# westlake-moonlight/vision_transformer_detector

Hardware: AMD Instinct MI355X
Metric: images/sec ViT-B/16 detector fwd, batch 256, 1/2/4/8 MI355X; MFMA util % (higher is better)
Workload: dtype bf16; 1 GPU; vit_b16_224 detector forward + decode; per_gpu_batch=256, global_batch=256, parallelism=dp1, streams_per_gpu=2, hip_graph=False

## Files before the change

### vision_transformer_detector_amd/csrc/vtd_gemm.hip

```cpp
#include <stdlib.h>

#include <algorithm>
#include <mutex>
#include <type_traits>

#include "vtd_common.h"
#include "vtd_gemm_epi.h"
#include "vtd_launch.h"

namespace vtd {

namespace {

constexpr int BM = 128, BN = 128, KB = 128;
constexpr int NT = 256;
constexpr int TILE_BYTES = BM * KB;


__device__ __forceinline__ int swz(int row, int chunk) {
  return row * KB + ((chunk ^ (row & 7)) << 4);
}


__device__ __forceinline__ void gload4(i32x4 (&ra)[4], i32x4 (&rb)[4], const char* ga,
// ... 166 lines not shown
#pragma unroll
        for (int cb = 0; cb < 2; ++cb) {
          const int r = 16 * cb + fr, c = 4 * (sb & 1) + g;
          const bf16x8 b = *reinterpret_cast<const bf16x8*>(smem + (sb >> 1) * 4096 + r * 128 +
                                                            ((c ^ (r & 7)) << 4));
          acc[cb] = __builtin_amdgcn_mfma_f32_16x16x32_bf16(__builtin_bit_cast(bf16x8, a[j]), b,
                                                            acc[cb], 0, 0, 0);
        }
      }
    }
  };
  for (int s0 = 0; s0 < nks; s0 += 2 * SK_CH) {
    if (s0 + SK_CH < nks) load(a1, s0 + SK_CH);
    compute(a0, s0);
    if (s0 + 2 * SK_CH < nks) load(a0, s0 + 2 * SK_CH);
    if (s0 + SK_CH < nks) compute(a1, s0 + SK_CH);
  }
#pragma unroll
  for (int cb = 0; cb < 2; ++cb)
#pragma unroll
    for (int r = 0; r < 4; ++r) epi_store(e, M, N, m0 + 4 * g + r, n0 + 16 * cb + fr, acc[cb][r]);
}

constexpr int BBM = 256, BBN = 256, BNT = 512;
#ifndef VTD_TRS
#define VTD_TRS 0
#endif
#ifndef VTD_PP2_PH
#define VTD_PP2_PH 2
#endif
constexpr int BSTAGE = (BBM + BBN) * KB;
static_assert(8 * 32 * 68 * 4 + 8 * 128 * 8 <= 2 * BSTAGE,
              "epilogue staging + LayerNorm-fold row tables must fit the stages");

typedef __attribute__((address_space(3))) void lds_void_t;
typedef __attribute__((address_space(1))) const void gbl_void_t;


struct NoPF {
  __device__ void operator()() const {}
};

template <int O0, int O1, int O2, int O3>
__device__ __forceinline__ void lds_read4_b64(const void* p, float2 (&o)[4]) {
  const uint32_t a = static_cast<uint32_t>(reinterpret_cast<uintptr_t>(p));
  asm volatile(
      "ds_read_b64 %0, %4 offset:%5\n\tds_read_b64 %1, %4 offset:%6\n\t"
      "ds_read_b64 %2, %4 offset:%7\n\tds_read_b64 %3, %4 offset:%8\n\ts_waitcnt lgkmcnt(0)"
      : "=v"(o[0]), "=v"(o[1]), "=v"(o[2]), "=v"(o[3])
      : "v"(a), "i"(O0), "i"(O1), "i"(O2), "i"(O3)
      : "memory");
}
__device__ __forceinline__ void store_s3(const EpiArgs& e, int64_t idx, const i32x4& o, f32x4 v0,
                                         f32x4 v1) {
  const i32x4 lo = {(int)pack_lo_bf16x2(v0[0], v0[1], (uint32_t)o[0]),
                    (int)pack_lo_bf16x2(v0[2], v0[3], (uint32_t)o[1]),
                    (int)pack_lo_bf16x2(v1[0], v1[1], (uint32_t)o[2]),
                    (int)pack_lo_bf16x2(v1[2], v1[3], (uint32_t)o[3])};
  bf16_t* p = static_cast<bf16_t*>(e.out) + idx;
  store_out16(p + e.s3, lo);
}
template <int EPI, int PR = 32, int DG = 0, typename PF = NoPF, bool TRL = false>
__device__ __forceinline__ void epilogue_fast(const f32x4 (&acc)[8][4], float* ep, int lane,
                                              int m_base, int n_base, const EpiArgs& e,
                                              const float2* lst = nullptr, PF pf = PF{}) {
  constexpr int ACT = EPI & 3;
  constexpr bool OUT_BF16 = (EPI & 4) != 0;
  constexpr bool RESID = (EPI & 8) != 0 && !(DG & 2);
  constexpr bool NOBIAS = (EPI & EPI_PARTIAL) != 0;
  constexpr bool LNF = (EPI & EPI_LNF) != 0, STAT = (EPI & EPI_STAT) != 0 && !(DG & 1);
  constexpr bool F8O = (EPI & EPI_F8O) != 0;
  auto sidx = [](int row, int col) { return row * 64 + (((col >> 2) ^ (row & 7)) << 2) + (col & 3); };
  constexpr int NB = PR / 16;
  constexpr int NIT = PR / 8;
  const int fr = lane & 15, fg = lane >> 4;
  const int c8 = (lane & 7) * 8, rsub = lane >> 3;
  f32x4 b0 = {}, b1 = {};
  if constexpr (!NOBIAS) {
    b0 = *reinterpret_cast<const f32x4*>(e.bias + n_base + c8);
    b1 = *reinterpret_cast<const f32x4*>(e.bias + n_base + c8 + 4);
  }
  f32x4 cs0 = {}, cs1 = {};
  if constexpr (LNF) {
    cs0 = *reinterpret_cast<const f32x4*>(e.colsum + n_base + c8);
    cs1 = *reinterpret_cast<const f32x4*>(e.colsum + n_base + c8 + 4);
  }
  constexpr bool RPRE = RESID && OUT_BF16;
  i32x4 rraw[2][NIT];
  auto load_raw = [&](int pp, i32x4 (&dst)[NIT]) {
#pragma unroll
    for (int it = 0; it < NIT; ++it) {
      const int64_t m = m_base + pp * PR + it * 8 + rsub;
      dst[it] = *reinterpret_cast<const i32x4*>(static_cast<const bf16_t*>(e.resid) + m * e.ldr +
                                                n_base + c8);
    }
  };
  if constexpr (RPRE) load_raw(0, rraw[0]);
  else pf();
#pragma unroll
  for (int p = 0; p < 128 / PR; ++p) {
    if constexpr (TRL) {
#pragma unroll
      for (int i = 0; i < NB; ++i)
#pragma unroll
        for (int jj = 0; jj < 4; ++jj)
          *reinterpret_cast<f32x4*>(ep + sidx(i * 16 + fr, 32 * (jj >> 1) + 8 * fg + 4 * (jj & 1))) =
              acc[p * NB + i][jj];
    } else {
#pragma unroll
      for (int i = 0; i < NB; ++i)
#pragma unroll
        for (int j = 0; j < 4; ++j)
#pragma unroll
          for (int r2 = 0; r2 < 4; ++r2)
            ep[sidx(i * 16 + fg * 4 + r2, j * 16 + fr)] = acc[p * NB + i][j][r2];
    }
    if constexpr (RPRE) {
      if (p + 1 < 128 / PR) load_raw(p + 1, rraw[(p + 1) & 1]);
      if (p == 0) pf();
    }
    constexpr bool ASM_ST = LNF && !std::is_same<PF, NoPF>::value;
    float2 stv[4];
    if constexpr (ASM_ST) {
      static_assert(PR == 32, "the fold's table reads assume 32-row passes");
      if (p == 0) lds_read4_b64<0, 64, 128, 192>(lst + rsub, stv);
      else if (p == 1) lds_read4_b64<256, 320, 384, 448>(lst + rsub, stv);
      else if (p == 2) lds_read4_b64<512, 576, 640, 704>(lst + rsub, stv);
      else lds_read4_b64<768, 832, 896, 960>(lst + rsub, stv);
    }
    f32x4 rv[NIT][2];
    [[maybe_unused]] float2 stkeep = float2{0.f, 0.f};
    if constexpr (RESID && !RPRE) {
#pragma unroll
      for (int it = 0; it < NIT; ++it) {
        const int64_t m = m_base + p * PR + it * 8 + rsub;
        load_resid8<OUT_BF16>(e, m * e.ldr + n_base + c8, rv[it][0], rv[it][1]);
      }
    }
#pragma unroll
    for (int it = 0; it < NIT; ++it) {
      const int row = it * 8 + rsub;
      f32x4 v0 = *reinterpret_cast<const f32x4*>(ep + sidx(row, c8));
      f32x4 v1 = *reinterpret_cast<const f32x4*>(ep + sidx(row, c8 + 4));
      if constexpr (ASM_ST) epi_lnfold8_st(stv[it], cs0, cs1, v0, v1);
      else if constexpr (LNF) epi_lnfold8_st(lst[p * PR + row], cs0, cs1, v0, v1);
      v0 += b0;
      v1 += b1;
      if constexpr ((EPI & EPI_RA) != 0) epi_rowadd8(e, m_base + p * PR + row, n_base + c8, v0, v1);
      act_ct8<ACT>(v0, v1);
      if constexpr (RPRE) {
        const i32x4 w = rraw[p & 1][it];
        v0 += bf16x4_to_f32((uint32_t)w[0], (uint32_t)w[1]);
        v1 += bf16x4_to_f32((uint32_t)w[2], (uint32_t)w[3]);
      } else if constexpr (RESID) {
        v0 += rv[it][0];
        v1 += rv[it][1];
      }
      if constexpr ((EPI & EPI_O2) != 0) epi_out2_8(e, m_base + p * PR + row, n_base + c8, v0, v1);
      const int64_t idx = (int64_t)(m_base + p * PR + row) * e.ldo + n_base + c8;
      if constexpr (OUT_BF16) {
        if constexpr (F8O) {
          bf16_round4(v0);
          bf16_round4(v1);
          float am = 0.f;
#pragma unroll
          for (int j = 0; j < 4; ++j) am = fmaxf(am, fmaxf(fabsf(v0[j]), fabsf(v1[j])));
          am = fmaxf(am, dpp_f32<0xB1>(am));
          am = fmaxf(am, dpp_f32<0x4E>(am));
          const int E = mx8_exponent(am);
          const float inv = __uint_as_float((uint32_t)(127 - E) << 23);
          const uint2 qv = {mx8_pack4(v0[0], v0[1], v0[2], v0[3], inv),
                            mx8_pack4(v1[0], v1[1], v1[2], v1[3], inv)};
          *reinterpret_cast<uint2*>(static_cast<uint8_t*>(e.out) + idx) = qv;
          if ((lane & 3) == 0) {
            const int n = n_base + c8, b = n >> 5;
            e.sout[((int64_t)(b >> 2) * e.s_rows + m_base + p * PR + row) * 4 + (b & 3)] =
                (uint8_t)(E + 127);
          }
          continue;
        }
        const i32x4 o = {(int)pack_bf16x2(v0[0], v0[1]), (int)pack_bf16x2(v0[2], v0[3]),
                         (int)pack_bf16x2(v1[0], v1[1]), (int)pack_bf16x2(v1[2], v1[3])};
        if constexpr (DG & 4) asm volatile("" ::"v"(o));
        else store_out16(static_cast<bf16_t*>(e.out) + idx, o);
        if constexpr ((EPI & EPI_S3) != 0) store_s3(e, idx, o, v0, v1);
        if constexpr (STAT) {
          f32x2 pv[4];
          bf16x8_unpack(o, pv);
          const float mean = sum8_dpp(pairs_sum(pv)) * (1.f / 64.f);
          const float m2 = sum8_dpp(pairs_m2(pv, mean));
          if ((lane & 7) == it) stkeep = float2{mean, m2};
        }
      } else {
        float* op = static_cast<float*>(e.out) + idx;
        *reinterpret_cast<f32x4*>(op) = v0;
        *reinterpret_cast<f32x4*>(op + 4) = v1;
      }
    }
    if constexpr (OUT_BF16 && STAT && !F8O) {
      static_assert(NIT <= 8, "one statistics row per lane of an 8-lane group");
      if ((lane & 7) < NIT)
        e.statout[(int64_t)(n_base >> 6) * e.stat_ld + m_base + p * PR + (lane & 7) * 8 + rsub] =
            stkeep;
    }
  }
}
template <int PR = 32>
__device__ __forceinline__ void epilogue_generic_pass(const float* ep, int lane, int M, int N,
                                                      int m_base, int n_base, const EpiArgs& e) {
  constexpr int ES = 68;
#pragma unroll 1
  for (int it = 0; it < PR / 4; ++it) {
    const int row = it * 4 + (lane >> 4), col = (lane & 15) * 4;
    const f32x4 v = *reinterpret_cast<const f32x4*>(ep + row * ES + col);
    epi_store4(e, M, N, m_base + row, n_base + col, v);
  }
}
// ... 247 lines not shown
    else pp_mfma<4, 2, F32>(acc, a, b1);
    if constexpr (!NB) pp_barrier();
    if constexpr (n2) {
      pp2_issue<2, AW>(smem, src, wave, kt + 2, kt & 1);
      pp2_issue<3, AW>(smem, src, wave, kt + 2, kt & 1);
      asm volatile("s_waitcnt vmcnt(10)" ::: "memory");
    } else {
      asm volatile("s_waitcnt vmcnt(0)" ::: "memory");
    }
    if constexpr (!NB) pp_barrier();
    if constexpr (TR) pp_mfma_t<4, 0, F32>(acc, a, b0);
    else pp_mfma<4, 0, F32>(acc, a, b0);
    if constexpr (!NB) pp_barrier();
  };
  int kt = 0;
  for (; kt + 2 < nk; ++kt) step(kt, std::true_type{}, std::true_type{});
  if (kt + 1 < nk) step(kt++, std::true_type{}, std::false_type{});
  step(kt, std::false_type{}, std::false_type{});
  if (wm == 0) pp_barrier();
}

template <int I0, bool TR, bool F32>
__device__ __forceinline__ void pp_mfma32(f32x4 (&acc)[8][4], const bf16x8 (&a)[4][2],
                                          const bf16x8 (&b0)[2][2], const bf16x8 (&b1)[2][2]) {
  if constexpr (TR) {
    pp_mfma_t<I0, 0, F32>(acc, a, b0);
    pp_mfma_t<I0, 2, F32>(acc, a, b1);
  } else {
    pp_mfma<I0, 0, F32>(acc, a, b0);
    pp_mfma<I0, 2, F32>(acc, a, b1);
  }
}

template <bool AW>
__device__ __forceinline__ void pp2_issue_first(char* smem, const PP2Src<AW>& src, int nk,
                                                int wave) {
  pp2_issue<0, AW>(smem, src, wave, 0, 0);
  pp2_issue<2, AW>(smem, src, wave, 0, 0);
  pp2_issue<3, AW>(smem, src, wave, 0, 0);
  pp2_issue<1, AW>(smem, src, wave, 0, 0);
  if (nk > 1) {
    pp2_issue<0, AW>(smem, src, wave, 1, 1);
    pp2_issue<2, AW>(smem, src, wave, 1, 1);
    pp2_issue<3, AW>(smem, src, wave, 1, 1);
  }
}

template <bool TR, bool F32 = false, bool AW = true, int EX = 0>
__device__ __forceinline__ void pp2_mainloop_2ph(f32x4 (&acc)[8][4], char* smem,
                                                 const PP2Src<AW>& src, int nk, int wave, int wm,
                                                 int wn, int fr, int fg,
                                                 uint64_t* t_prologue = nullptr) {
  if (nk > 1) asm volatile("s_waitcnt vmcnt(%0)" ::"i"(6 + EX) : "memory");
  else asm volatile("s_waitcnt vmcnt(%0)" ::"i"(EX) : "memory");
  pp_barrier();
  if (t_prologue) *t_prologue = __builtin_amdgcn_s_memtime();
  if (wm == 1) pp_barrier();
  const int ra = wm * 64, rb = wn * 32;
  bf16x8 a[4][2], b0[2][2], b1[2][2];
  auto step = [&](int kt, auto t1, auto t2, auto ex) {
    const char* st = smem + (kt & 1) * BSTAGE;
    constexpr bool n1 = decltype(t1)::value, n2 = decltype(t2)::value;
    constexpr int W8 = 8 + decltype(ex)::value;
    pp_load_a(a, st + 0 * 16384, ra, fr, fg);
    if constexpr (TR) {
      pp_load_b_t(b0, st + 2 * 16384, rb, fr, fg);
// ... 4 lines not shown
    }
    if constexpr (n1) {
      pp2_issue<1, AW>(smem, src, wave, kt + 1, (kt + 1) & 1);
      asm volatile("s_waitcnt vmcnt(%0)" ::"i"(W8) : "memory");
    } else {
      asm volatile("s_waitcnt vmcnt(0)" ::: "memory");
    }
    pp_barrier();
    pp_mfma32<0, TR, F32>(acc, a, b0, b1);
    pp_barrier();
    pp_load_a(a, st + 1 * 16384, ra, fr, fg);
    if constexpr (n2) {
      pp2_issue<0, AW>(smem, src, wave, kt + 2, kt & 1);
      pp2_issue<2, AW>(smem, src, wave, kt + 2, kt & 1);
      pp2_issue<3, AW>(smem, src, wave, kt + 2, kt & 1);
      asm volatile("s_waitcnt vmcnt(%0)" ::"i"(W8) : "memory");
    } else {
      asm volatile("s_waitcnt vmcnt(0) lgkmcnt(0)" ::: "memory");
    }
    pp_barrier();
    pp_mfma32<4, TR, F32>(acc, a, b0, b1);
    if (n1 || n2 || wm == 0) pp_barrier();
  };
  constexpr std::integral_constant<int, 0> ex0{};
  int kt = 0;
  if constexpr (EX > 0) {
    if (nk > 2) step(kt++, std::true_type{}, std::true_type{}, std::integral_constant<int, EX>{});
  }
  for (; kt + 2 < nk; ++kt) step(kt, std::true_type{}, std::true_type{}, ex0);
  if (kt + 1 < nk) step(kt++, std::true_type{}, std::false_type{}, ex0);
  step(kt, std::false_type{}, std::false_type{}, ex0);
}

template <int EPI, int DG = 0, typename PF = NoPF>
__device__ __forceinline__ void epilogue_direct(const f32x4 (&acc)[8][4], int lane, int m_base,
                                                int n_base, const EpiArgs& e,
                                                const float2* lst = nullptr, PF pf = PF{}) {
  constexpr int ACT = EPI & 3;
  constexpr bool OUT_BF16 = (EPI & 4) != 0;
  constexpr bool RESID = (EPI & 8) != 0 && !(DG & 2);
  constexpr bool LNF = (EPI & EPI_LNF) != 0, STAT = (EPI & EPI_STAT) != 0 && !(DG & 1);
  constexpr bool F8O = (EPI & EPI_F8O) != 0;
  static_assert(!(F8O && (STAT || (EPI & EPI_S3) != 0)), "MX-fp8 output: no statistics / split");
  const int fr = lane & 15, fg = lane >> 4;
  f32x4 bias[2][2], cs[2][2] = {};
#pragma unroll
  for (int jp = 0; jp < 2; ++jp)
#pragma unroll
    for (int h = 0; h < 2; ++h) {
      bias[jp][h] = *reinterpret_cast<const f32x4*>(e.bias + n_base + 32 * jp + 8 * fg + 4 * h);
      if constexpr (LNF)
        cs[jp][h] = *reinterpret_cast<const f32x4*>(e.colsum + n_base + 32 * jp + 8 * fg + 4 * h);
    }
  constexpr bool RPRE = RESID && OUT_BF16;
  i32x4 rraw[2][4][2];
  auto load_raw = [&](int h0, i32x4 (&dst)[4][2]) {
#pragma unroll
    for (int i = 0; i < 4; ++i)
#pragma unroll
      for (int jp = 0; jp < 2; ++jp)
        dst[i][jp] = *reinterpret_cast<const i32x4*>(
            static_cast<const bf16_t*>(e.resid) + (int64_t)(m_base + 16 * (h0 + i) + fr) * e.ldr +
            n_base + 32 * jp + 8 * fg);
  };
  if constexpr (RPRE) load_raw(0, rraw[0]);
  else pf();
#pragma unroll
  for (int i0 = 0; i0 < 8; i0 += 4) {
    f32x4 rv[4][2][2];
    float2 st[4];
    if constexpr (LNF && !std::is_same<PF, NoPF>::value) {
      if (i0 == 0) lds_read4_b64<0, 128, 256, 384>(lst + fr, st);
      else lds_read4_b64<512, 640, 768, 896>(lst + fr, st);
    } else if constexpr (LNF) {
#pragma unroll
      for (int i = 0; i < 4; ++i) st[i] = lst[16 * (i0 + i) + fr];
    }
    [[maybe_unused]] float2 stkeep = float2{0.f, 0.f};
    if constexpr (RPRE) {
      if (i0 == 0) {
        load_raw(4, rraw[1]);
        pf();
      }
    } else if constexpr (RESID) {
#pragma unroll
      for (int i = 0; i < 4; ++i)
#pragma unroll
        for (int jp = 0; jp < 2; ++jp) {
          load_resid8<OUT_BF16>(e, (int64_t)(m_base + 16 * (i0 + i) + fr) * e.ldr + n_base +
                                       32 * jp + 8 * fg, rv[i][jp][0], rv[i][jp][1]);
        }
    }
#pragma unroll
    for (int i = 0; i < 4; ++i) {
      float tsum = 0.f;
      i32x4 ob[2];
#pragma unroll
      for (int jp = 0; jp < 2; ++jp) {
        f32x4 v0 = acc[i0 + i][2 * jp];
// ... 8 lines not shown
        if constexpr (RPRE) {
          const i32x4 w = rraw[i0 >> 2][i][jp];
          v0 += bf16x4_to_f32((uint32_t)w[0], (uint32_t)w[1]);
          v1 += bf16x4_to_f32((uint32_t)w[2], (uint32_t)w[3]);
        } else if constexpr (RESID) {
          v0 += rv[i][jp][0];
          v1 += rv[i][jp][1];
        }
        if constexpr ((EPI & EPI_O2) != 0) epi_out2_8(e, mrow, ncol, v0, v1);
        const int64_t idx = (int64_t)mrow * e.ldo + ncol;
        if constexpr (F8O) {
          bf16_round4(v0);
          bf16_round4(v1);
          float am = 0.f;
#pragma unroll
          for (int j = 0; j < 4; ++j) am = fmaxf(am, fmaxf(fabsf(v0[j]), fabsf(v1[j])));
          am = xmax32(xmax16(am));
          const int E = mx8_exponent(am);
          const float inv = __uint_as_float((uint32_t)(127 - E) << 23);
          const uint2 qv = {mx8_pack4(v0[0], v0[1], v0[2], v0[3], inv),
                            mx8_pack4(v1[0], v1[1], v1[2], v1[3], inv)};
          *reinterpret_cast<uint2*>(static_cast<uint8_t*>(e.out) + idx) = qv;
          if (fg == 0) {
            const int b = (n_base + 32 * jp) >> 5;
            e.sout[((int64_t)(b >> 2) * e.s_rows + mrow) * 4 + (b & 3)] = (uint8_t)(E + 127);
          }
          continue;
        }
        if constexpr (OUT_BF16) {
          const i32x4 o = {(int)pack_bf16x2(v0[0], v0[1]), (int)pack_bf16x2(v0[2], v0[3]),
                           (int)pack_bf16x2(v1[0], v1[1]), (int)pack_bf16x2(v1[2], v1[3])};
          if constexpr (DG & 4) asm volatile("" ::"v"(o));
          else store_out16(static_cast<bf16_t*>(e.out) + idx, o);
          if constexpr ((EPI & EPI_S3) != 0) store_s3(e, idx, o, v0, v1);
          if constexpr (STAT) {
            ob[jp] = o;
            tsum += bf16x8_sum(o);
          }
        } else {
          float* op = static_cast<float*>(e.out) + idx;
          *reinterpret_cast<f32x4*>(op) = v0;
          *reinterpret_cast<f32x4*>(op + 4) = v1;
        }
      }
      if constexpr (OUT_BF16 && STAT) {
        const float mean = xsum32(xsum16(tsum)) * (1.f / 64.f);
        const float m2 = xsum32(xsum16(bf16x8_m2(ob[0], mean) + bf16x8_m2(ob[1], mean)));
        if (fg == i) stkeep = float2{mean, m2};
      }
    }
    if constexpr (OUT_BF16 && STAT)
      e.statout[(int64_t)(n_base >> 6) * e.stat_ld + m_base + 16 * (i0 + fg) + fr] = stkeep;
  }
}

__device__ __forceinline__ void epilogue_direct_generic(const f32x4 (&acc)[8][4], float* ep,
                                                        int lane, int M, int N, int m_base,
                                                        int n_base, const EpiArgs& e) {
  constexpr int ES = 68;
  const int fr = lane & 15, fg = lane >> 4;
#pragma unroll
  for (int p = 0; p < 4; ++p) {
#pragma unroll
    for (int i = 0; i < 2; ++i)
#pragma unroll
      for (int jj = 0; jj < 4; ++jj)
        *reinterpret_cast<f32x4*>(ep + (i * 16 + fr) * ES + 32 * (jj >> 1) + 8 * fg +
                                  4 * (jj & 1)) = acc[p * 2 + i][jj];
    epilogue_generic_pass<32>(ep, lane, M, N, m_base + p * 32, n_base, e);
  }
}

#if VTD_DIAG
constexpr int kStampSlots = 16384;
__device__ uint64_t g_pp2_stamps[kStampSlots * 6];
#endif

template <int EPI, bool TR = false, int DG = 0>
__global__ __launch_bounds__(BNT) void gemm_tn_bf16_pp2_kernel(
    int M, int N, int K, const bf16_t* __restrict__ A, int lda,
    const bf16_t* __restrict__ Bt, int ldb, int tiles_m, int tiles_n, EpiArgs e, int ksplit) {
  extern __shared__ __attribute__((aligned(16))) char smem[];
  const int tid = threadIdx.x;
  const int lane = tid & 63;
  const int wave = __builtin_amdgcn_readfirstlane(tid >> 6);
  const int wm = wave >> 2, wn = wave & 3;
  uint64_t ts[4] = {0, 0, 0, 0};
  [[maybe_unused]] uint64_t rt0 = 0;
  if constexpr ((DG & 16) != 0) {
    ts[0] = __builtin_amdgcn_s_memtime();
    rt0 = __builtin_amdgcn_s_memrealtime();
  }
  asm volatile("" ::"s"(M), "s"(N), "s"(K), "s"(A), "s"(lda), "s"(Bt), "s"(ldb), "s"(tiles_m),
               "s"(tiles_n), "s"(ksplit), "s"(e.to.tiles_n), "s"(e.to.grouped), "s"(e.aw));
  const int nt = tiles_m * tiles_n, nwg = nt * ksplit;
  const int bid = blockIdx.x;
#if VTD_DIAG
  if (e.dsl > 0 && bid < 256 && ((bid >> 3) & 1))
    for (int i = 0; i < e.dsl; ++i) __builtin_amdgcn_s_sleep(8);
#endif
  const int xcd = bid & 7, q = nwg >> 3, r = nwg & 7;
  const int v = xcd * q + min(xcd, r) + (bid >> 3);
  const int split = ksplit > 1 ? v / nt : 0, tile = v - split * nt;
  int tm, tn;
  tile_coords(tile, e.to, tm, tn);
  const int m0 = tm * BBM, n0 = tn * BBN;
  const int nk_all = K / 64, nks = ksplit > 1 ? (nk_all + ksplit - 1) / ksplit : nk_all;
  const int k0 = split * nks, nk = min(nks, nk_all - k0);
  PP2Src<pp2_wraps(EPI)> src;
  pp2b_sources<TR>(src, A, lda, M, Bt, ldb, N, m0, n0, wave, lane, k0 * 64, true, e.aw);
  constexpr bool kEarly = VTD_PP2_PH == 2 && (DG & 32) == 0;
  constexpr bool kLnf = EPI != EPI_GENERIC && (EPI & EPI_LNF) != 0;
  if constexpr (kEarly) {
    pp2_issue_first(smem, src, nk, wave);
    __builtin_amdgcn_sched_barrier(0);
    asm volatile("" ::: "memory");
  }
  if (ksplit > 1) e.out = static_cast<float*>(e.out) + split * e.split_stride;
  float2 lst[2] = {float2{0.f, 0.f}, float2{0.f, 0.f}};
  if constexpr (kLnf) {
    lst[0] = e.lnstat[min(m0 + wm * 128 + lane, M - 1)];
    lst[1] = e.lnstat[min(m0 + wm * 128 + 64 + lane, M - 1)];
  }
  f32x4 acc[8][4];
#pragma unroll
  for (int i = 0; i < 8; ++i)
#pragma unroll
    for (int j = 0; j < 4; ++j) {
      acc[i][j] = f32x4{0.f, 0.f, 0.f, 0.f};
      if constexpr (kEarly) asm volatile("" : "+v"(acc[i][j]));
    }
  const int fr = lane & 15, fg = lane >> 4;
  if constexpr (kEarly)
    pp2_mainloop_2ph<TR, false, pp2_wraps(EPI), kLnf ? 2 : 0>(acc, smem, src, nk, wave, wm, wn, fr,
                                                             fg, (DG & 16) ? &ts[1] : nullptr);
  else
    pp2_mainloop<TR, false, (DG & 32) != 0>(acc, smem, src, nk, wave, wm, wn, fr, fg,
                                             (DG & 16) ? &ts[1] : nullptr);
  if constexpr ((DG & 16) != 0) ts[2] = __builtin_amdgcn_s_memtime();
  const int m_base = m0 + wm * 128, n_base = n0 + wn * 64;
#if VTD_DIAG
  auto stamp = [&]() {
    if constexpr ((DG & 16) != 0) {
      ts[3] = __builtin_amdgcn_s_memtime();
      if (wave == 0 && lane == 0 && bid < kStampSlots) {
        g_pp2_stamps[bid * 6 + 0] = ts[0];
        g_pp2_stamps[bid * 6 + 1] = ts[1];
        g_pp2_stamps[bid * 6 + 2] = ts[2];
        g_pp2_stamps[bid * 6 + 3] = ts[3];
        g_pp2_stamps[bid * 6 + 4] = rt0;
        g_pp2_stamps[bid * 6 + 5] = __builtin_amdgcn_s_memrealtime();
      }
    }
  };
#else
  auto stamp = [&]() {};
#endif
  float2* const lds_st = reinterpret_cast<float2*>(smem + 8 * 32 * 68 * 4) + wave * 128;
  if constexpr (EPI != EPI_GENERIC && (EPI & EPI_LNF) != 0) {
    lds_st[lane] = lst[0];
    lds_st[64 + lane] = lst[1];
  }
  if constexpr ((DG & 8) != 0) {
#pragma unroll
    for (int i = 0; i < 8; ++i)
#pragma unroll
      for (int j = 0; j < 4; ++j) asm volatile("" ::"v"(acc[i][j]));
    return;
  }
  if constexpr (TR) {
    if constexpr (EPI != EPI_GENERIC) {
      if (m0 + BBM <= M && n0 + BBN <= N) {
        if constexpr (VTD_TRS && (EPI & 4) != 0 && (EPI & EPI_F8O) == 0)
          epilogue_fast<EPI, 32, DG, NoPF, true>(acc, reinterpret_cast<float*>(smem) + wave * 32 * 68,
                                                 lane, m_base, n_base, e, lds_st);
        else
          epilogue_direct<EPI, DG>(acc, lane, m_base, n_base, e, lds_st);
        stamp();
        return;
      }
    }
    epilogue_direct_generic(acc, reinterpret_cast<float*>(smem) + wave * 32 * 68, lane, M, N,
                            m_base, n_base, e);
    return;
  }
  float* ep = reinterpret_cast<float*>(smem) + wave * 32 * 68;
  if constexpr (EPI != EPI_GENERIC) {
    if (m0 + BBM <= M && n0 + BBN <= N) {
      epilogue_fast<EPI, 32, DG>(acc, ep, lane, m_base, n_base, e, lds_st);
      stamp();
      return;
    }
  }
  epilogue_generic(acc, ep, lane, M, N, m_base, n_base, e);
}

#if VTD_DIAG
template <int EPI, bool TR>
__global__ __launch_bounds__(BNT) void gemm_tn_bf16_pp2_mt_kernel(
    int M, int N, int K, const bf16_t* __restrict__ A, int lda,
    const bf16_t* __restrict__ Bt, int ldb, int tiles_m, int tiles_n, EpiArgs e) {
  constexpr int DG = 0;
  extern __shared__ __attribute__((aligned(16))) char smem[];
  const int tid = threadIdx.x;
  const int lane0 = tid & 63;
  const int wave = __builtin_amdgcn_readfirstlane(tid >> 6);
  const int wm = wave >> 2, wn = wave & 3;
  const int nt = tiles_m * tiles_n;
  const int nwg = gridDim.x;
  const int bid = blockIdx.x;
  const int xcd = bid & 7, q = nwg >> 3, r = nwg & 7;
  const int v = (xcd < r ? xcd * (q + 1) : r * (q + 1) + (xcd - r) * q) + (bid >> 3);
  int tile = v;
  const int nk = K / 64, k0 = 0;
  int tm, tn;
  tile_coords(tile, e.to, tm, tn);
  char* const epb = smem + BSTAGE;
  uint64_t ts[4] = {0, 0, 0, 0};
  [[maybe_unused]] uint64_t rt0 = 0;
  if constexpr ((DG & 16) != 0) {
    ts[0] = __builtin_amdgcn_s_memtime();
    rt0 = __builtin_amdgcn_s_memrealtime();
// ... 374 lines not shown
  auto a16 = [](const void* p) { return reinterpret_cast<uintptr_t>(p) % 16 == 0; };
  if (!(dtype == VTD_BF16 && e->out_dtype == VTD_BF16 && tiles >= kMinBigTiles && N > 64 &&
        M % BBM == 0 && N % BBN == 0 && e->bias && e->statout &&
        e->scatter_tokens <= 0 && e->ldo % 8 == 0 && a16(e->out) && a16(e->bias) &&
        (!e->resid || (e->ldr % 8 == 0 && a16(e->resid))) &&
        (!e->out2 || (e->ldo2 % 8 == 0 && a16(e->out2))) && e->stat_ld >= M &&
        reinterpret_cast<uintptr_t>(e->statout) % 8 == 0))
    return false;
  return (pp2_code(e) & EPI_STAT) != 0 && pp2_code(e) != EPI_GENERIC;
}

constexpr int kSkinnyMaxN = 320;
bool skinny_choice(int M, int N, int K) {
  const int kn = knob(VTD_KNOB_SKINNY);
  const int max_n = kn >= 64 ? kn : kSkinnyMaxN;
  return kn != 0 && N <= max_n && K % 64 == 0 && M > 0;
}

bool gemm_mx8_emits_fp8(int M, int N, const vtd_epilogue* e) {
  auto a16 = [](const void* p) { return reinterpret_cast<uintptr_t>(p) % 16 == 0; };
  return M % BBM == 0 && N % BBN == 0 && e->bias && a16(e->bias) && !e->resid && !e->rowadd &&
         !e->out2 && e->scatter_tokens <= 0 && !e->lnstat && e->ldo % 16 == 0 && a16(e->out) &&
         e->scale_out && e->scale_rows >= M && e->scale_rows % 4 == 0;
}

constexpr size_t kPP2LdsMax = BSTAGE + 8 * 32 * 68 * 4 + 8 * 128 * 8;
static_assert(kPP2LdsMax <= 160 * 1024 && kPP2LdsMax >= 2 * BSTAGE, "pp2 LDS");
constexpr bool pp2_mt_code(int c) {
  return c == (4 | EPI_LNF) || c == (5 | EPI_LNF) || c == (12 | EPI_STAT) || c == 5 || c == 12;
}
inline int pp2_tpw() { return std::max(1, knob(VTD_KNOB_GEMM_TPW)); }

template <int C>
void pp2_launch(bool tr, dim3 g, hipStream_t stream, int M, int N, int K, const bf16_t* A, int lda,
                const bf16_t* Bt, int ldb, int tiles_m, int tiles_n, const EpiArgs& e,
                int ksplit = 1) {
#if VTD_DIAG
  if constexpr (pp2_mt_code(C)) {
    if (ksplit == 1 && e.tpw > 1) {
      const dim3 gm((tiles_m * tiles_n + e.tpw - 1) / e.tpw);
      if (tr)
        hipLaunchKernelGGL((gemm_tn_bf16_pp2_mt_kernel<C, true>), gm, dim3(BNT), kPP2LdsMax,
                           stream, M, N, K, A, lda, Bt, ldb, tiles_m, tiles_n, e);
      else
        hipLaunchKernelGGL((gemm_tn_bf16_pp2_mt_kernel<C, false>), gm, dim3(BNT), kPP2LdsMax,
                           stream, M, N, K, A, lda, Bt, ldb, tiles_m, tiles_n, e);
      return;
    }
  }
#endif
  if (tr)
    hipLaunchKernelGGL((gemm_tn_bf16_pp2_kernel<C, true>), g, dim3(BNT), 2 * BSTAGE, stream, M,
                       N, K, A, lda, Bt, ldb, tiles_m, tiles_n, e, ksplit);
  else
    hipLaunchKernelGGL((gemm_tn_bf16_pp2_kernel<C, false>), g, dim3(BNT), 2 * BSTAGE, stream, M,
                       N, K, A, lda, Bt, ldb, tiles_m, tiles_n, e, ksplit);
}

void pp2_set_attributes() {
  static std::once_flag once[kMaxDevices];
  once_per_device(once, [] {
#define VTD_PP_FN(C) reinterpret_cast<const void*>(&gemm_tn_bf16_pp2_kernel<C, false>), \
                     reinterpret_cast<const void*>(&gemm_tn_bf16_pp2_kernel<C, true>),
    const void* fns[] = {VTD_PP_FN(EPI_GENERIC) VTD_PP2_CODES(VTD_PP_FN)};
#undef VTD_PP_FN
    for (const void* f : fns)
      (void)hipFuncSetAttribute(f, hipFuncAttributeMaxDynamicSharedMemorySize, 2 * BSTAGE);
#if VTD_DIAG
#define VTD_MT_FN(C) reinterpret_cast<const void*>(&gemm_tn_bf16_pp2_mt_kernel<C, false>), \
                     reinterpret_cast<const void*>(&gemm_tn_bf16_pp2_mt_kernel<C, true>),
    const void* mts[] = {VTD_MT_FN(4 | EPI_LNF) VTD_MT_FN(5 | EPI_LNF) VTD_MT_FN(12 | EPI_STAT)
                         VTD_MT_FN(5) VTD_MT_FN(12)};
#undef VTD_MT_FN
    for (const void* f : mts)
      (void)hipFuncSetAttribute(f, hipFuncAttributeMaxDynamicSharedMemorySize, (int)kPP2LdsMax);
#endif
  });
}

__global__ __launch_bounds__(256) void gemm_splitk_epilogue_kernel(
    const float* __restrict__ part, int ksplit, int64_t stride, int M, int N, int ldp,
    EpiArgs e) {
  const int nq = (N + 3) >> 2;
  const int64_t i = (int64_t)blockIdx.x * 256 + threadIdx.x;
  if (i >= (int64_t)M * nq) return;
  const int m = (int)(i / nq), n = (int)(i - (int64_t)m * nq) * 4;
  const float* p = part + (int64_t)m * ldp + n;
  f32x4 v = *reinterpret_cast<const f32x4*>(p);
  for (int s = 1; s < ksplit; ++s) v += *reinterpret_cast<const f32x4*>(p + s * stride);
  epi_store4(e, M, N, m, n, v);
}

#define VTD_F32_CODES(X) X(0) X(1) X(2) X(8) X(9) X(10) X(EPI_RA)
void f32_pp2_launch(int M, int N, int K, const float* A, int lda, const float* Bt, int ldb,
                    const vtd_epilogue* epi, int tiles_m, int tiles_n, hipStream_t stream) {
  static std::once_flag once[kMaxDevices];
  once_per_device(once, [] {
#define VTD_F32_FN(C) reinterpret_cast<const void*>(&gemm_tn_f32_pp2_kernel<C, false>), \
                      reinterpret_cast<const void*>(&gemm_tn_f32_pp2_kernel<C, true>),
    const void* fns[] = {VTD_F32_FN(EPI_GENERIC) VTD_F32_CODES(VTD_F32_FN)};
// ... 77 lines not shown
    const char* v = getenv("VTD_SMALL_PP2");
    return !v || atoi(v) != 0;
  }();
  const bool big = tiles_m * tiles_n >= kMinBigTiles && N > 64;
  const bool skinny = dtype == VTD_BF16 && K - 32 * aw <= SK_KMAX && skinny_choice(M, N, K);
  const bool few = small_pp2 && N > 64 && !skinny;
  if (dtype == VTD_BF16 && (big || few)) {
    const bf16_t* a16 = static_cast<const bf16_t*>(A);
    const bf16_t* b16 = static_cast<const bf16_t*>(Bt);
    const int ngw = tile_group_width(tiles_n);
#if VTD_DIAG
    if (gemm_variant() == 12 && epi->out_dtype != VTD_BF16X3 && aw == 0) {
      if (!gemm_w4_launch(M, N, K, a16, lda, b16, ldb, epi, ngw, stream))
        return fail(VTD_ERR_HIP, "gemm: w4 kernel attributes could not be set");
      VTD_LAUNCH_CHECK("gemm");
      return VTD_OK;
    }
#endif
    pp2_set_attributes();
    EpiArgs e = make_epi_args(epi);
    e.aw = aw;
    e.ngw = ngw;
    e.to = make_tile_order(tiles_m, tiles_n, e.ngw);
    e.tpw = VTD_DIAG ? pp2_tpw() : 1;
#if VTD_DIAG
    static const int pp2_sleep = getenv("VTD_PP2_SLEEP") ? atoi(getenv("VTD_PP2_SLEEP")) : 0;
    e.dsl = pp2_sleep;
#endif
    const int code = aw > 0 && !pp2_wraps(pp2_code(epi)) ? EPI_GENERIC : pp2_code(epi);
    const int ktr = knob(VTD_KNOB_GEMM_TR);
    const bool tr = ktr >= 0 ? ktr != 0 : e.act != VTD_ACT_NONE;
    const dim3 g(tiles_m * tiles_n);
#if VTD_DIAG
    const size_t lds = 2 * BSTAGE;
    static const int pp2_dg = getenv("VTD_PP2_DG") ? atoi(getenv("VTD_PP2_DG")) : 0;
    if (pp2_dg > 0 && aw == 0) {
      bool done = true;
      auto dg = [&](auto c) {
        constexpr int C = decltype(c)::value;
        static std::once_flag once[kMaxDevices];
        once_per_device(once, [] {
          for (const void* f : {reinterpret_cast<const void*>(&gemm_tn_bf16_pp2_kernel<C, false, 1>),
                                reinterpret_cast<const void*>(&gemm_tn_bf16_pp2_kernel<C, true, 1>),
                                reinterpret_cast<const void*>(&gemm_tn_bf16_pp2_kernel<C, false, 2>),
                                reinterpret_cast<const void*>(&gemm_tn_bf16_pp2_kernel<C, true, 2>),
                                reinterpret_cast<const void*>(&gemm_tn_bf16_pp2_kernel<C, false, 4>),
                                reinterpret_cast<const void*>(&gemm_tn_bf16_pp2_kernel<C, true, 4>),
                                reinterpret_cast<const void*>(&gemm_tn_bf16_pp2_kernel<C, false, 8>),
                                reinterpret_cast<const void*>(&gemm_tn_bf16_pp2_kernel<C, true, 8>),
                                reinterpret_cast<const void*>(&gemm_tn_bf16_pp2_kernel<C, false, 16>),
                                reinterpret_cast<const void*>(&gemm_tn_bf16_pp2_kernel<C, true, 16>),
                                reinterpret_cast<const void*>(&gemm_tn_bf16_pp2_kernel<C, false, 32>),
                                reinterpret_cast<const void*>(&gemm_tn_bf16_pp2_kernel<C, true, 32>)})
            (void)hipFuncSetAttribute(f, hipFuncAttributeMaxDynamicSharedMemorySize, 2 * BSTAGE);
        });
#define VTD_DG_L(D)                                                                                \
  if (pp2_dg == D) {                                                                               \
    if (tr) hipLaunchKernelGGL((gemm_tn_bf16_pp2_kernel<C, true, D>), g, dim3(BNT), lds,           \
                               stream, M, N, K, a16, lda, b16, ldb, tiles_m, tiles_n, e, 1);       \
    else hipLaunchKernelGGL((gemm_tn_bf16_pp2_kernel<C, false, D>), g, dim3(BNT), lds,             \
                            stream, M, N, K, a16, lda, b16, ldb, tiles_m, tiles_n, e, 1);          \
  }
        VTD_DG_L(1) VTD_DG_L(2) VTD_DG_L(4) VTD_DG_L(8) VTD_DG_L(16) VTD_DG_L(32)
#undef VTD_DG_L
      };
      switch (code) {
        case 4: dg(std::integral_constant<int, 4>{}); break;
        case 5: dg(std::integral_constant<int, 5>{}); break;
        case 12: dg(std::integral_constant<int, 12>{}); break;
        case 13: dg(std::integral_constant<int, 13>{}); break;
        case 12 | EPI_STAT: dg(std::integral_constant<int, 12 | EPI_STAT>{}); break;
        case 13 | EPI_STAT: dg(std::integral_constant<int, 13 | EPI_STAT>{}); break;
        case 4 | EPI_LNF: dg(std::integral_constant<int, 4 | EPI_LNF>{}); break;
        case 5 | EPI_LNF: dg(std::integral_constant<int, 5 | EPI_LNF>{}); break;
        default: done = false;
      }
      if (done) {
        VTD_LAUNCH_CHECK("gemm");
        return VTD_OK;
      }
    }
#endif
    switch (code) {
#define VTD_PP_CASE(C) \
  case C: pp2_launch<C>(tr, g, stream, M, N, K, a16, lda, b16, ldb, tiles_m, tiles_n, e); break;
      VTD_PP2_CODES(VTD_PP_CASE)
#undef VTD_PP_CASE
      default:
        pp2_launch<EPI_GENERIC>(tr, g, stream, M, N, K, a16, lda, b16, ldb, tiles_m, tiles_n, e);
    }
  } else if (dtype == VTD_F32 && big && knob(VTD_KNOB_F32_PP2) != 0) {
    f32_pp2_launch(M, N, K, static_cast<const float*>(A), lda, static_cast<const float*>(Bt), ldb,
                   epi, tiles_m, tiles_n, stream);
// ... 195 lines not shown
                        void* stream) {
  return vtd::gemm_launch(M, N, K, A_dev, lda, Bt_dev, ldb, dtype, epi,
                          static_cast<hipStream_t>(stream), 0.0);
}

extern "C" int vtd_gemm_mx8(int M, int N, int K, const uint8_t* A_dev, int lda,
                            const uint8_t* sA_dev, int64_t sa_rows, const uint8_t* Bt_dev,
                            int ldb, const uint8_t* sB_dev, int64_t sb_rows,
                            const vtd_epilogue* epi, void* stream) {
  return vtd::gemm_mx8_launch(M, N, K, A_dev, lda, sA_dev, sa_rows, Bt_dev, ldb, sB_dev, sb_rows,
                              epi, static_cast<hipStream_t>(stream), 0.0);
}

extern "C" int vtd_gemm_splitk(int M, int N, int K, const void* A_dev, int lda,
                               const void* Bt_dev, int ldb, int dtype, const vtd_epilogue* epi,
                               float* part_dev, size_t part_bytes, int ksplit, void* stream) {
  if (ksplit < 2 || part_bytes < (size_t)ksplit * (size_t)std::max(M, 0) * std::max(N, 0) * 4)
    return vtd::fail(VTD_ERR_INVALID_ARG, "gemm_splitk: ksplit < 2 or part_bytes too small");
  return vtd::gemm_splitk_launch(M, N, K, A_dev, lda, Bt_dev, ldb, dtype, epi, part_dev, ksplit,
                                 static_cast<hipStream_t>(stream), 0.0);
}

extern "C" int vtd_gemm_splitk_choice(int M, int N, int K, int dtype) {
  return vtd::gemm_splitk_choice(M, N, K, dtype, 0);
}

#if VTD_DIAG
extern "C" int vtd_diag_build(void) { return 1; }
extern "C" int vtd_diag_read_stamps(uint64_t* host, int n) {
  n = std::min(n, vtd::kStampSlots);
  return hipMemcpyFromSymbol(host, HIP_SYMBOL(vtd::g_pp2_stamps), (size_t)n * 6 * 8, 0,
                             hipMemcpyDeviceToHost) == hipSuccess ? 0 : -3;
}
#endif
```

Before: 21100 images/s.

## Prefetch epilogue bias, colsum and LN stats into LDS edge area during prologue

```diff
diff --git a/vision_transformer_detector_amd/csrc/vtd_gemm.hip b/vision_transformer_detector_amd/csrc/vtd_gemm.hip
--- a/vision_transformer_detector_amd/csrc/vtd_gemm.hip
+++ b/vision_transformer_detector_amd/csrc/vtd_gemm.hip
@@ -222,6 +222,18 @@
 constexpr int BSTAGE = (BBM + BBN) * KB;
 static_assert(8 * 32 * 68 * 4 + 8 * 128 * 8 <= 2 * BSTAGE,
               "epilogue staging + LayerNorm-fold row tables must fit the stages");
+#ifndef VTD_PP2_EDGE
+#define VTD_PP2_EDGE 1
+#endif
+constexpr int kEdgeBias = 0, kEdgeColsum = 1024, kEdgeStat = 2048;
+constexpr bool pp2_edge_bias(int code) { return code != EPI_GENERIC && (code & EPI_PARTIAL) == 0; }
+constexpr bool pp2_edge_fold(int code) { return pp2_edge_bias(code) && (code & EPI_LNF) != 0; }
+constexpr int pp2_edge_bytes(int code) {
+  return pp2_edge_fold(code) ? kEdgeStat + 8 * 128 * 8 : pp2_edge_bias(code) ? kEdgeStat : 0;
+}
+constexpr int kPP2EdgeMax = kEdgeStat + 8 * 128 * 8;
+static_assert(2 * BSTAGE + kPP2EdgeMax <= 160 * 1024 && 2 * (2 * BSTAGE) > 160 * 1024,
+              "pp2 stages + edge area: one workgroup per CU, within the CU's 160 KiB");
 
 typedef __attribute__((address_space(3))) void lds_void_t;
 typedef __attribute__((address_space(1))) const void gbl_void_t;
@@ -230,6 +242,16 @@
 struct NoPF {
   __device__ void operator()() const {}
 };
+
+#if VTD_DIAG
+constexpr int kStampSlots = 16384;
+__device__ uint64_t g_pp2_stamps[kStampSlots * 6];
+__device__ uint64_t g_pp2_store_stamps[kStampSlots];
+__device__ __forceinline__ void pp2_store_stamp() {
+  if (threadIdx.x == 0 && blockIdx.x < kStampSlots)
+    g_pp2_store_stamps[blockIdx.x] = __builtin_amdgcn_s_memtime();
+}
+#endif
 
 template <int O0, int O1, int O2, int O3>
 __device__ __forceinline__ void lds_read4_b64(const void* p, float2 (&o)[4]) {
@@ -241,6 +263,26 @@
       : "v"(a), "i"(O0), "i"(O1), "i"(O2), "i"(O3)
       : "memory");
 }
+template <int O0, int O1, int O2, int O3>
+__device__ __forceinline__ void lds_read4_b128(const void* p, f32x4& o0, f32x4& o1, f32x4& o2,
+                                               f32x4& o3) {
+  const uint32_t a = static_cast<uint32_t>(reinterpret_cast<uintptr_t>(p));
+  asm volatile(
+      "ds_read_b128 %0, %4 offset:%5\n\tds_read_b128 %1, %4 offset:%6\n\t"
+      "ds_read_b128 %2, %4 offset:%7\n\tds_read_b128 %3, %4 offset:%8\n\ts_waitcnt lgkmcnt(0)"
+      : "=&v"(o0), "=&v"(o1), "=&v"(o2), "=v"(o3)
+      : "v"(a), "i"(O0), "i"(O1), "i"(O2), "i"(O3)
+      : "memory");
+}
+template <int O0, int O1>
+__device__ __forceinline__ void lds_read2_b128(const void* p, f32x4& o0, f32x4& o1) {
+  const uint32_t a = static_cast<uint32_t>(reinterpret_cast<uintptr_t>(p));
+  asm volatile("ds_read_b128 %0, %2 offset:%3\n\tds_read_b128 %1, %2 offset:%4\n\t"
+               "s_waitcnt lgkmcnt(0)"
+               : "=&v"(o0), "=v"(o1)
+               : "v"(a), "i"(O0), "i"(O1)
+               : "memory");
+}
 __device__ __forceinline__ void store_s3(const EpiArgs& e, int64_t idx, const i32x4& o, f32x4 v0,
                                          f32x4 v1) {
   const i32x4 lo = {(int)pack_lo_bf16x2(v0[0], v0[1], (uint32_t)o[0]),
@@ -250,10 +292,12 @@
   bf16_t* p = static_cast<bf16_t*>(e.out) + idx;
   store_out16(p + e.s3, lo);
 }
-template <int EPI, int PR = 32, int DG = 0, typename PF = NoPF, bool TRL = false>
+template <int EPI, int PR = 32, int DG = 0, typename PF = NoPF, bool TRL = false,
+          bool EDGE = false>
 __device__ __forceinline__ void epilogue_fast(const f32x4 (&acc)[8][4], float* ep, int lane,
                                               int m_base, int n_base, const EpiArgs& e,
-                                              const float2* lst = nullptr, PF pf = PF{}) {
+                                              const float2* lst = nullptr, PF pf = PF{},
+                                              const float* edge = nullptr) {
   constexpr int ACT = EPI & 3;
   constexpr bool OUT_BF16 = (EPI & 4) != 0;
   constexpr bool RESID = (EPI & 8) != 0 && !(DG & 2);
@@ -266,14 +310,18 @@
   const int fr = lane & 15, fg = lane >> 4;
   const int c8 = (lane & 7) * 8, rsub = lane >> 3;
   f32x4 b0 = {}, b1 = {};
-  if constexpr (!NOBIAS) {
-    b0 = *reinterpret_cast<const f32x4*>(e.bias + n_base + c8);
-    b1 = *reinterpret_cast<const f32x4*>(e.bias + n_base + c8 + 4);
-  }
   f32x4 cs0 = {}, cs1 = {};
-  if constexpr (LNF) {
-    cs0 = *reinterpret_cast<const f32x4*>(e.colsum + n_base + c8);
-    cs1 = *reinterpret_cast<const f32x4*>(e.colsum + n_base + c8 + 4);
+  if constexpr (EDGE) {
+    static_assert(!NOBIAS, "the edge area holds a bias");
+  } else {
+    if constexpr (!NOBIAS) {
+      b0 = *reinterpret_cast<const f32x4*>(e.bias + n_base + c8);
+      b1 = *reinterpret_cast<const f32x4*>(e.bias + n_base + c8 + 4);
+    }
+    if constexpr (LNF) {
+      cs0 = *reinterpret_cast<const f32x4*>(e.colsum + n_base + c8);
+      cs1 = *reinterpret_cast<const f32x4*>(e.colsum + n_base + c8 + 4);
+    }
   }
   constexpr bool RPRE = RESID && OUT_BF16;
   i32x4 rraw[2][NIT];
@@ -308,6 +356,14 @@
     if constexpr (RPRE) {
       if (p + 1 < 128 / PR) load_raw(p + 1, rraw[(p + 1) & 1]);
       if (p == 0) pf();
+    }
+    if constexpr (EDGE) {
+      if (p == 0) {
+        if constexpr (LNF)
+          lds_read4_b128<0, 16, kEdgeColsum, kEdgeColsum + 16>(edge + c8, b0, b1, cs0, cs1);
+        else
+          lds_read2_b128<0, 16>(edge + c8, b0, b1);
+      }
     }
     constexpr bool ASM_ST = LNF && !std::is_same<PF, NoPF>::value;
     float2 stv[4];
@@ -373,6 +429,11 @@
                          (int)pack_bf16x2(v1[0], v1[1]), (int)pack_bf16x2(v1[2], v1[3])};
         if constexpr (DG & 4) asm volatile("" ::"v"(o));
         else store_out16(static_cast<bf16_t*>(e.out) + idx, o);
+#if VTD_DIAG
+        if constexpr ((DG & 16) != 0) {
+          if (p == 0 && it == 0) pp2_store_stamp();
+        }
+#endif
         if constexpr ((EPI & EPI_S3) != 0) store_s3(e, idx, o, v0, v1);
         if constexpr (STAT) {
           f32x2 pv[4];
@@ -686,6 +747,29 @@
   }
 }
 
+constexpr int pp2_edge_loads(int code) { return pp2_edge_fold(code) ? 3 : pp2_edge_bias(code) ? 1 : 0; }
+template <int EPI>
+__device__ __forceinline__ void pp2_issue_edge_cols(char* edge, const EpiArgs& e, int N, int n0,
+                                                    int wave, int lane) {
+  const int bytes = min(N - n0, BBN) * 4;
+  if (lane < 8) {
+    __builtin_amdgcn_raw_ptr_buffer_load_lds(
+        __builtin_amdgcn_make_buffer_rsrc(const_cast<float*>(e.bias + n0), 0, bytes, 0x00020000),
+        (lds_void_t*)(edge + kEdgeBias + wave * 128), 16, wave * 128 + lane * 16, 0, 0, 0);
+    if constexpr (pp2_edge_fold(EPI))
+      __builtin_amdgcn_raw_ptr_buffer_load_lds(
+          __builtin_amdgcn_make_buffer_rsrc(const_cast<float*>(e.colsum + n0), 0, bytes, 0x00020000),
+          (lds_void_t*)(edge + kEdgeColsum + wave * 128), 16, wave * 128 + lane * 16, 0, 0, 0);
+  }
+}
+__device__ __forceinline__ void pp2_issue_edge_rows(char* edge, const EpiArgs& e, int M, int m0,
+                                                    int wave, int wm, int lane) {
+  __builtin_amdgcn_raw_ptr_buffer_load_lds(
+      __builtin_amdgcn_make_buffer_rsrc(const_cast<float2*>(e.lnstat + m0), 0,
+                                        min(M - m0, BBM) * 8, 0x00020000),
+      (lds_void_t*)(edge + kEdgeStat + wave * 1024), 16, wm * 1024 + lane * 16, 0, 0, 0);
+}
+
 template <bool AW>
 __device__ __forceinline__ void pp2_issue_first(char* smem, const PP2Src<AW>& src, int nk,
                                                 int wave) {
@@ -756,10 +840,11 @@
   step(kt, std::false_type{}, std::false_type{}, ex0);
 }
 
-template <int EPI, int DG = 0, typename PF = NoPF>
+template <int EPI, int DG = 0, typename PF = NoPF, bool EDGE = false>
 __device__ __forceinline__ void epilogue_direct(const f32x4 (&acc)[8][4], int lane, int m_base,
                                                 int n_base, const EpiArgs& e,
-                                                const float2* lst = nullptr, PF pf = PF{}) {
+                                                const float2* lst = nullptr, PF pf = PF{},
+                                                const float* edge = nullptr) {
   constexpr int ACT = EPI & 3;
   constexpr bool OUT_BF16 = (EPI & 4) != 0;
   constexpr bool RESID = (EPI & 8) != 0 && !(DG & 2);
@@ -768,14 +853,16 @@
   static_assert(!(F8O && (STAT || (EPI & EPI_S3) != 0)), "MX-fp8 output: no statistics / split");
   const int fr = lane & 15, fg = lane >> 4;
   f32x4 bias[2][2], cs[2][2] = {};
-#pragma unroll
-  for (int jp = 0; jp < 2; ++jp)
-#pragma unroll
-    for (int h = 0; h < 2; ++h) {
-      bias[jp][h] = *reinterpret_cast<const f32x4*>(e.bias + n_base + 32 * jp + 8 * fg + 4 * h);
-      if constexpr (LNF)
-        cs[jp][h] = *reinterpret_cast<const f32x4*>(e.colsum + n_base + 32 * jp + 8 * fg + 4 * h);
-    }
+  if constexpr (!EDGE) {
+#pragma unroll
+    for (int jp = 0; jp < 2; ++jp)
+#pragma unroll
+      for (int h = 0; h < 2; ++h) {
+        bias[jp][h] = *reinterpret_cast<const f32x4*>(e.bias + n_base + 32 * jp + 8 * fg + 4 * h);
+        if constexpr (LNF)
+          cs[jp][h] = *reinterpret_cast<const f32x4*>(e.colsum + n_base + 32 * jp + 8 * fg + 4 * h);
+      }
+  }
   constexpr bool RPRE = RESID && OUT_BF16;
   i32x4 rraw[2][4][2];
   auto load_raw = [&](int h0, i32x4 (&dst)[4][2]) {
@@ -789,6 +876,12 @@
   };
   if constexpr (RPRE) load_raw(0, rraw[0]);
   else pf();
+  if constexpr (EDGE) {
+    lds_read4_b128<0, 16, 128, 144>(edge + 8 * fg, bias[0][0], bias[0][1], bias[1][0], bias[1][1]);
+    if constexpr (LNF)
+      lds_read4_b128<kEdgeColsum, kEdgeColsum + 16, kEdgeColsum + 128, kEdgeColsum + 144>(
+          edge + 8 * fg, cs[0][0], cs[0][1], cs[1][0], cs[1][1]);
+  }
 #pragma unroll
   for (int i0 = 0; i0 < 8; i0 += 4) {
     f32x4 rv[4][2][2];
@@ -863,6 +956,11 @@
                            (int)pack_bf16x2(v1[0], v1[1]), (int)pack_bf16x2(v1[2], v1[3])};
           if constexpr (DG & 4) asm volatile("" ::"v"(o));
           else store_out16(static_cast<bf16_t*>(e.out) + idx, o);
+#if VTD_DIAG
+          if constexpr ((DG & 16) != 0) {
+            if (i0 == 0 && i == 0 && jp == 0) pp2_store_stamp();
+          }
+#endif
           if constexpr ((EPI & EPI_S3) != 0) store_s3(e, idx, o, v0, v1);
           if constexpr (STAT) {
             ob[jp] = o;
@@ -902,10 +1000,6 @@
   }
 }
 
-#if VTD_DIAG
-constexpr int kStampSlots = 16384;
-__device__ uint64_t g_pp2_stamps[kStampSlots * 6];
-#endif
 
 template <int EPI, bool TR = false, int DG = 0>
 __global__ __launch_bounds__(BNT) void gemm_tn_bf16_pp2_kernel(
@@ -942,14 +1036,19 @@
   pp2b_sources<TR>(src, A, lda, M, Bt, ldb, N, m0, n0, wave, lane, k0 * 64, true, e.aw);
   constexpr bool kEarly = VTD_PP2_PH == 2 && (DG & 32) == 0;
   constexpr bool kLnf = EPI != EPI_GENERIC && (EPI & EPI_LNF) != 0;
+  constexpr bool kEdge = kEarly && VTD_PP2_EDGE && pp2_edge_bias(EPI);
+  constexpr bool kEdgeRows = kEdge && pp2_edge_fold(EPI);
+  char* const edge = smem + 2 * BSTAGE;
   if constexpr (kEarly) {
     pp2_issue_first(smem, src, nk, wave);
+    if constexpr (kEdge) pp2_issue_edge_cols<EPI>(edge, e, N, n0, wave, lane);
+    if constexpr (kEdgeRows) pp2_issue_edge_rows(edge, e, M, m0, wave, wm, lane);
     __builtin_amdgcn_sched_barrier(0);
     asm volatile("" ::: "memory");
   }
   if (ksplit > 1) e.out = static_cast<float*>(e.out) + split * e.split_stride;
-  float2 lst[2] = {float2{0.f, 0.f}, float2{0.f, 0.f}};
-  if constexpr (kLnf) {
+  [[maybe_unused]] float2 lst[2] = {float2{0.f, 0.f}, float2{0.f, 0.f}};
+  if constexpr (kLnf && !kEdgeRows) {
     lst[0] = e.lnstat[min(m0 + wm * 128 + lane, M - 1)];
     lst[1] = e.lnstat[min(m0 + wm * 128 + 64 + lane, M - 1)];
   }
@@ -963,8 +1062,8 @@
     }
   const int fr = lane & 15, fg = lane >> 4;
   if constexpr (kEarly)
-    pp2_mainloop_2ph<TR, false, pp2_wraps(EPI), kLnf ? 2 : 0>(acc, smem, src, nk, wave, wm, wn, fr,
-                                                             fg, (DG & 16) ? &ts[1] : nullptr);
+    pp2_mainloop_2ph<TR, false, pp2_wraps(EPI), kEdge ? pp2_edge_loads(EPI) : kLnf ? 2 : 0>(
+        acc, smem, src, nk, wave, wm, wn, fr, fg, (DG & 16) ? &ts[1] : nullptr);
   else
     pp2_mainloop<TR, false, (DG & 32) != 0>(acc, smem, src, nk, wave, wm, wn, fr, fg,
                                              (DG & 16) ? &ts[1] : nullptr);
@@ -987,11 +1086,13 @@
 #else
   auto stamp = [&]() {};
 #endif
-  float2* const lds_st = reinterpret_cast<float2*>(smem + 8 * 32 * 68 * 4) + wave * 128;
-  if constexpr (EPI != EPI_GENERIC && (EPI & EPI_LNF) != 0) {
+  float2* const lds_st =
+      reinterpret_cast<float2*>(kEdgeRows ? edge + kEdgeStat : smem + 8 * 32 * 68 * 4) + wave * 128;
+  if constexpr (kLnf && !kEdgeRows) {
     lds_st[lane] = lst[0];
     lds_st[64 + lane] = lst[1];
   }
+  const float* const edge_w = reinterpret_cast<const float*>(edge + kEdgeBias) + wn * 64;
   if constexpr ((DG & 8) != 0) {
 #pragma unroll
     for (int i = 0; i < 8; ++i)
@@ -1003,10 +1104,11 @@
     if constexpr (EPI != EPI_GENERIC) {
       if (m0 + BBM <= M && n0 + BBN <= N) {
         if constexpr (VTD_TRS && (EPI & 4) != 0 && (EPI & EPI_F8O) == 0)
-          epilogue_fast<EPI, 32, DG, NoPF, true>(acc, reinterpret_cast<float*>(smem) + wave * 32 * 68,
-                                                 lane, m_base, n_base, e, lds_st);
+          epilogue_fast<EPI, 32, DG, NoPF, true, kEdge>(
+              acc, reinterpret_cast<float*>(smem) + wave * 32 * 68, lane, m_base, n_base, e, lds_st,
+              NoPF{}, edge_w);
         else
-          epilogue_direct<EPI, DG>(acc, lane, m_base, n_base, e, lds_st);
+          epilogue_direct<EPI, DG, NoPF, kEdge>(acc, lane, m_base, n_base, e, lds_st, NoPF{}, edge_w);
         stamp();
         return;
       }
@@ -1018,7 +1120,8 @@
   float* ep = reinterpret_cast<float*>(smem) + wave * 32 * 68;
   if constexpr (EPI != EPI_GENERIC) {
     if (m0 + BBM <= M && n0 + BBN <= N) {
-      epilogue_fast<EPI, 32, DG>(acc, ep, lane, m_base, n_base, e, lds_st);
+      epilogue_fast<EPI, 32, DG, NoPF, false, kEdge>(acc, ep, lane, m_base, n_base, e, lds_st, NoPF{},
+                                                     edge_w);
       stamp();
       return;
     }
@@ -1459,6 +1562,9 @@
 inline int pp2_tpw() { return std::max(1, knob(VTD_KNOB_GEMM_TPW)); }
 
 template <int C>
+constexpr size_t kPP2Lds = 2 * BSTAGE + (VTD_PP2_PH == 2 && VTD_PP2_EDGE ? pp2_edge_bytes(C) : 0);
+
+template <int C>
 void pp2_launch(bool tr, dim3 g, hipStream_t stream, int M, int N, int K, const bf16_t* A, int lda,
                 const bf16_t* Bt, int ldb, int tiles_m, int tiles_n, const EpiArgs& e,
                 int ksplit = 1) {
@@ -1477,10 +1583,10 @@
   }
 #endif
   if (tr)
-    hipLaunchKernelGGL((gemm_tn_bf16_pp2_kernel<C, true>), g, dim3(BNT), 2 * BSTAGE, stream, M,
+    hipLaunchKernelGGL((gemm_tn_bf16_pp2_kernel<C, true>), g, dim3(BNT), kPP2Lds<C>, stream, M,
                        N, K, A, lda, Bt, ldb, tiles_m, tiles_n, e, ksplit);
   else
-    hipLaunchKernelGGL((gemm_tn_bf16_pp2_kernel<C, false>), g, dim3(BNT), 2 * BSTAGE, stream, M,
+    hipLaunchKernelGGL((gemm_tn_bf16_pp2_kernel<C, false>), g, dim3(BNT), kPP2Lds<C>, stream, M,
                        N, K, A, lda, Bt, ldb, tiles_m, tiles_n, e, ksplit);
 }
 
@@ -1492,7 +1598,8 @@
     const void* fns[] = {VTD_PP_FN(EPI_GENERIC) VTD_PP2_CODES(VTD_PP_FN)};
 #undef VTD_PP_FN
     for (const void* f : fns)
-      (void)hipFuncSetAttribute(f, hipFuncAttributeMaxDynamicSharedMemorySize, 2 * BSTAGE);
+      (void)hipFuncSetAttribute(f, hipFuncAttributeMaxDynamicSharedMemorySize,
+                                2 * BSTAGE + kPP2EdgeMax);
 #if VTD_DIAG
 #define VTD_MT_FN(C) reinterpret_cast<const void*>(&gemm_tn_bf16_pp2_mt_kernel<C, false>), \
                      reinterpret_cast<const void*>(&gemm_tn_bf16_pp2_mt_kernel<C, true>),
@@ -1636,7 +1743,6 @@
     const bool tr = ktr >= 0 ? ktr != 0 : e.act != VTD_ACT_NONE;
     const dim3 g(tiles_m * tiles_n);
 #if VTD_DIAG
-    const size_t lds = 2 * BSTAGE;
     static const int pp2_dg = getenv("VTD_PP2_DG") ? atoi(getenv("VTD_PP2_DG")) : 0;
     if (pp2_dg > 0 && aw == 0) {
       bool done = true;
@@ -1656,13 +1762,14 @@
                                 reinterpret_cast<const void*>(&gemm_tn_bf16_pp2_kernel<C, true, 16>),
                                 reinterpret_cast<const void*>(&gemm_tn_bf16_pp2_kernel<C, false, 32>),
                                 reinterpret_cast<const void*>(&gemm_tn_bf16_pp2_kernel<C, true, 32>)})
-            (void)hipFuncSetAttribute(f, hipFuncAttributeMaxDynamicSharedMemorySize, 2 * BSTAGE);
+            (void)hipFuncSetAttribute(f, hipFuncAttributeMaxDynamicSharedMemorySize,
+                                      2 * BSTAGE + kPP2EdgeMax);
         });
 #define VTD_DG_L(D)                                                                                \
   if (pp2_dg == D) {                                                                               \
-    if (tr) hipLaunchKernelGGL((gemm_tn_bf16_pp2_kernel<C, true, D>), g, dim3(BNT), lds,           \
+    if (tr) hipLaunchKernelGGL((gemm_tn_bf16_pp2_kernel<C, true, D>), g, dim3(BNT), kPP2Lds<C>,    \
                                stream, M, N, K, a16, lda, b16, ldb, tiles_m, tiles_n, e, 1);       \
-    else hipLaunchKernelGGL((gemm_tn_bf16_pp2_kernel<C, false, D>), g, dim3(BNT), lds,             \
+    else hipLaunchKernelGGL((gemm_tn_bf16_pp2_kernel<C, false, D>), g, dim3(BNT), kPP2Lds<C>,      \
                             stream, M, N, K, a16, lda, b16, ldb, tiles_m, tiles_n, e, 1);          \
   }
         VTD_DG_L(1) VTD_DG_L(2) VTD_DG_L(4) VTD_DG_L(8) VTD_DG_L(16) VTD_DG_L(32)
@@ -1924,4 +2031,9 @@
   return hipMemcpyFromSymbol(host, HIP_SYMBOL(vtd::g_pp2_stamps), (size_t)n * 6 * 8, 0,
                              hipMemcpyDeviceToHost) == hipSuccess ? 0 : -3;
 }
+extern "C" int vtd_diag_read_store_stamps(uint64_t* host, int n) {
+  n = std::min(n, vtd::kStampSlots);
+  return hipMemcpyFromSymbol(host, HIP_SYMBOL(vtd::g_pp2_store_stamps), (size_t)n * 8, 0,
+                             hipMemcpyDeviceToHost) == hipSuccess ? 0 : -3;
+}
 #endif
```

After: 21090 images/s. Within noise of the previous version (-0.0%).
